# facebookresearch/jepa

Measured on NVIDIA H100. Metric: clips/sec ViT-L/16 16x224^2 synthetic V-JEPA pre-training step, higher is better.
Workload: dtype bf16

## Files before the change

### jepa_b200/csrc/attn_bwd.cu

```cuda
#include <stdlib.h>

#include "attn_common.cuh"
#include "vjepa_b200.h"

namespace vj {

constexpr int kBwdStream = 64;
constexpr int kBwdStages = 3;

struct AttnBwdParams {
  const int* cu_seqlens;
  const float* lse2;
  const float* delta;
  __nv_bfloat16* dqkv;
  int H, T;
  float scale, scale_log2;
};

template <int HD, bool DKV>
constexpr int bwd_nwg() { return HD == 128 || (HD == 64 && DKV) ? 2 : (HD == 32 && !DKV) ? 4 : 3; }

template <int HD, int NWG>
struct BwdCfg {
  using A = AttnCfg<HD>;
  static constexpr int RES = A::template tile_bytes<AttnWarps<NWG>::ROWS>();
  static constexpr int STR = A::template tile_bytes<kBwdStream>();
  static constexpr int T0 = 0, T1 = RES;
  static constexpr int S_OFF = 2 * RES;
  static constexpr int STAT_OFF = S_OFF + kBwdStages * 2 * STR;
  static constexpr int STAT = 2 * kBwdStream * 4;
  static constexpr int BAR_OFF = STAT_OFF + kBwdStages * STAT;
  static constexpr int SMEM_BYTES = BAR_OFF + 8 * (1 + 2 * kBwdStages) + 1024;
  static_assert(SMEM_BYTES <= 232448, "attention backward shared memory budget exceeded");
};

__global__ void __launch_bounds__(256) attn_delta_kernel(const __nv_bfloat16* __restrict__ o,
                                                         const __nv_bfloat16* __restrict__ dout,
                                                         float* __restrict__ delta, int T, int H, int HD) {
  const int lane = threadIdx.x & 31;
  const int wpb = blockDim.x >> 5;
  const int D = H * HD;
  const int nvec = D >> 3;
  const int lanes_per_head = HD >> 3;
  for (long long t = (long long)blockIdx.x * wpb + (threadIdx.x >> 5); t < T; t += (long long)gridDim.x * wpb) {
    for (int c = lane; c < ((nvec + 31) / 32) * 32; c += 32) {
      float s = 0.f;
      if (c < nvec) {
        const uint4 a = *reinterpret_cast<const uint4*>(o + t * D + c * 8);
        const uint4 b = *reinterpret_cast<const uint4*>(dout + t * D + c * 8);
        s = bf16_lo(a.x) * bf16_lo(b.x) + bf16_hi(a.x) * bf16_hi(b.x) + bf16_lo(a.y) * bf16_lo(b.y) +
            bf16_hi(a.y) * bf16_hi(b.y) + bf16_lo(a.z) * bf16_lo(b.z) + bf16_hi(a.z) * bf16_hi(b.z) +
            bf16_lo(a.w) * bf16_lo(b.w) + bf16_hi(a.w) * bf16_hi(b.w);
      }
      for (int o2 = lanes_per_head >> 1; o2 > 0; o2 >>= 1) s += __shfl_xor_sync(0xffffffffu, s, o2);
      if (c < nvec && (lane % lanes_per_head) == 0) delta[(long long)((c * 8) / HD) * T + t] = s;
    }
  }
}

template <int HD, bool DKV, int NWG>
__global__ void __launch_bounds__(AttnWarps<NWG>::THREADS, 1)
attn_bwd_kernel(const __grid_constant__ CUtensorMap tmRes, const __grid_constant__ CUtensorMap tmStr,
                const __grid_constant__ CUtensorMap tmDO, const AttnBwdParams p) {
  using B = BwdCfg<HD, NWG>;
  using W = AttnWarps<NWG>;
  extern __shared__ uint8_t smem_raw[];
  uint8_t* smem = reinterpret_cast<uint8_t*>((reinterpret_cast<uintptr_t>(smem_raw) + 1023) & ~uintptr_t(1023));

  const int seq = blockIdx.y, head = blockIdx.z;
  const int row_begin = p.cu_seqlens[seq];
  const int len = p.cu_seqlens[seq + 1] - row_begin;
  const int t0 = blockIdx.x * W::ROWS;
  if (t0 >= len) return;
  const int n_wg = attn_active_wgs<NWG>(len, t0);
  const int n_it = (len + kBwdStream - 1) / kBwdStream;
  const int HHD = p.H * HD;

  uint64_t* bars = reinterpret_cast<uint64_t*>(smem + B::BAR_OFF);
  const uint32_t bar_res = smem_u32(bars + 0);
  const uint32_t full0 = smem_u32(bars + 1);
  const uint32_t empty0 = smem_u32(bars + 1 + kBwdStages);
  const uint32_t sT0 = smem_u32(smem + B::T0), sT1 = smem_u32(smem + B::T1), sS = smem_u32(smem + B::S_OFF);
  const uint32_t sStat = smem_u32(smem + B::STAT_OFF);
  const float* lse_h = p.lse2 + (long long)head * p.T + row_begin;
  const float* del_h = p.delta + (long long)head * p.T + row_begin;
  const int wg = __shfl_sync(0xffffffffu, threadIdx.x >> 7, 0);
  const int lane = threadIdx.x & 31;

  if (threadIdx.x == 0) {
    mbar_init(bar_res, 1);
    for (int st = 0; st < kBwdStages; ++st) {
      mbar_init(full0 + 8 * st, DKV ? 32 : 1);
      mbar_init(empty0 + 8 * st, 4 * n_wg);
    }
    fence_mbar_init();
  }
  __syncthreads();

  if (wg == 0) {
    setmaxnreg_dec<W::PRODUCER_REGS>();
    if (threadIdx.x < 32) {
      if (lane == 0) {
        mbar_expect_tx(bar_res, 2 * B::RES);
        if (DKV) {
          attn_load_tile<HD, W::ROWS>(sT0, &tmRes, bar_res, HHD + head * HD, row_begin + t0);
          attn_load_tile<HD, W::ROWS>(sT1, &tmRes, bar_res, 2 * HHD + head * HD, row_begin + t0);
        } else {
          attn_load_tile<HD, W::ROWS>(sT0, &tmRes, bar_res, head * HD, row_begin + t0);
          attn_load_tile<HD, W::ROWS>(sT1, &tmDO, bar_res, head * HD, row_begin + t0);
        }
      }
      for (int i = 0; i < n_it; ++i) {
        const int st = i % kBwdStages;
        const uint32_t a = sS + st * 2 * B::STR, b = a + B::STR, bar = full0 + 8 * st;
        const int c0 = i * kBwdStream;
        mbar_wait(empty0 + 8 * st, ((i / kBwdStages) & 1) ^ 1);
        if (DKV) {
#pragma unroll
          for (int k = 0; k < kBwdStream / 32; ++k) {
            const int col = c0 + 32 * k + lane;
            const uint32_t dst = sStat + st * B::STAT + (32 * k + lane) * 4;
            sts32f(dst, col < len ? lse_h[col] : 0.f);
            sts32f(dst + B::STAT / 2, col < len ? del_h[col] : 0.f);
          }
        }
        if (lane == 0) {
          mbar_expect_tx(bar, 2 * B::STR);
          if (DKV) {
            attn_load_tile<HD, kBwdStream>(a, &tmStr, bar, head * HD, row_begin + c0);
            attn_load_tile<HD, kBwdStream>(b, &tmDO, bar, head * HD, row_begin + c0);
          } else {
            attn_load_tile<HD, kBwdStream>(a, &tmStr, bar, HHD + head * HD, row_begin + c0);
            attn_load_tile<HD, kBwdStream>(b, &tmStr, bar, 2 * HHD + head * HD, row_begin + c0);
          }
        } else if (DKV) {
          mbar_arrive(bar);
        }
      }
    }
    return;
  }

  const int cw = wg - 1;
  if (cw >= n_wg) return;
  setmaxnreg_inc<W::CONSUMER_REGS>();
  const int r = cw * 64 + ((threadIdx.x >> 5) & 3) * 16 + (lane >> 2);
  float acc0[HD / 2], acc1[HD / 2];
#pragma unroll
  for (int i = 0; i < HD / 2; ++i) { acc0[i] = 0.f; acc1[i] = 0.f; }
  float row_lse[2], row_del[2];
  if (!DKV) {
#pragma unroll
    for (int h = 0; h < 2; ++h) {
      const int q = t0 + r + 8 * h;
      row_lse[h] = q < len ? lse_h[q] : 0.f;
      row_del[h] = q < len ? del_h[q] : 0.f;
    }
  }
  mbar_wait(bar_res, 0);
  for (int i = 0; i < n_it; ++i) {
    const int st = i % kBwdStages;
    const uint32_t sa = sS + st * 2 * B::STR, sb = sa + B::STR;
    const int c0 = i * kBwdStream;
    mbar_wait(full0 + 8 * st, (i / kBwdStages) & 1);
    float x[kBwdStream / 2], y[kBwdStream / 2];
    wgmma_fence();
#pragma unroll
    for (int kk = 0; kk < HD / 16; ++kk)
      wgmma_ss<kBwdStream, 0, 0>(x, attn_kmajor_desc<HD, W::ROWS>(sT0, cw * 64, kk), attn_kmajor_desc<HD, kBwdStream>(sa, 0, kk),
                                 kk > 0);
#pragma unroll
    for (int kk = 0; kk < HD / 16; ++kk)
      wgmma_ss<kBwdStream, 0, 0>(y, attn_kmajor_desc<HD, W::ROWS>(sT1, cw * 64, kk), attn_kmajor_desc<HD, kBwdStream>(sb, 0, kk),
                                 kk > 0);
    wgmma_commit();
    wgmma_wait<0>();
    wgmma_fence_regs(x);
    wgmma_fence_regs(y);

#pragma unroll
    for (int c = 0; c < kBwdStream / 8; ++c)
#pragma unroll
      for (int e = 0; e < 2; ++e) {
        const int col = 8 * c + 2 * (lane & 3) + e;
        const bool col_ok = c0 + col < len;
        float cl = 0.f, cd = 0.f;
        if (DKV) {
          cl = lds32f(sStat + st * B::STAT + col * 4);
          cd = lds32f(sStat + st * B::STAT + B::STAT / 2 + col * 4);
        }
#pragma unroll
        for (int h = 0; h < 2; ++h) {
          const float l2 = DKV ? cl : row_lse[h], dl = DKV ? cd : row_del[h];
          float& pv = x[4 * c + 2 * h + e];
          float& dv = y[4 * c + 2 * h + e];
          pv = col_ok ? ex2_approx(fmaf(pv, p.scale_log2, -l2)) : 0.f;
          dv = pv * (dv - dl);
        }
      }

    wgmma_fence_regs(acc0);
    wgmma_fence_regs(acc1);
    wgmma_fence();
#pragma unroll
    for (int kk = 0; kk < kBwdStream / 16; ++kk) {
      uint32_t a[4];
      if (DKV) {
        acc_to_afrag(x, kk, a);
        wgmma_rs<HD, 1>(acc0, a, attn_mnmajor_desc<HD, kBwdStream>(sb, kk), 1);
        acc_to_afrag(y, kk, a);
        wgmma_rs<HD, 1>(acc1, a, attn_mnmajor_desc<HD, kBwdStream>(sa, kk), 1);
      } else {
        acc_to_afrag(y, kk, a);
        wgmma_rs<HD, 1>(acc0, a, attn_mnmajor_desc<HD, kBwdStream>(sa, kk), 1);
      }
    }
    wgmma_commit();
    wgmma_wait<0>();
    wgmma_fence_regs(acc0);
    wgmma_fence_regs(acc1);
    __syncwarp();
    if (lane == 0) mbar_arrive(empty0 + 8 * st);
  }

  __nv_bfloat16* rows = p.dqkv + (long long)(row_begin + t0) * 3 * HHD + head * HD;
  if (DKV) {
    store_frag<HD>(acc1, p.scale, rows + HHD, 3LL * HHD, r, len - t0);
    store_frag<HD>(acc0, 1.0f, rows + 2 * HHD, 3LL * HHD, r, len - t0);
  } else {
    store_frag<HD>(acc0, p.scale, rows, 3LL * HHD, r, len - t0);
  }
}

template <int HD>
static int launch_attn_bwd(const void* qkv, const void* out, const void* dout, const float* lse2, float* delta,
                           void* dqkv, const int* cu, int nseq, int max_len, int H, int T, float scale, cudaStream_t s) {
  constexpr int NKV = bwd_nwg<HD, true>(), NQ = bwd_nwg<HD, false>();
  using C = AttnCfg<HD>;
  using BKV = BwdCfg<HD, NKV>;
  using BQ = BwdCfg<HD, NQ>;
  using WKV = AttnWarps<NKV>;
  using WQ = AttnWarps<NQ>;
  CUtensorMap tq_kv, tq_q, tdo_q, tq64, tdo64;
  const uint64_t W = (uint64_t)3 * H * HD, WO = (uint64_t)H * HD;
  int rc = make_tmap_2d(&tq_kv, qkv, 0, W, T, W * 2, C::BOX_INNER, WKV::ROWS, C::TMAP_SWIZZLE);
  if (!rc) rc = make_tmap_2d(&tq_q, qkv, 0, W, T, W * 2, C::BOX_INNER, WQ::ROWS, C::TMAP_SWIZZLE);
  if (!rc) rc = make_tmap_2d(&tq64, qkv, 0, W, T, W * 2, C::BOX_INNER, kBwdStream, C::TMAP_SWIZZLE);
  if (!rc) rc = make_tmap_2d(&tdo_q, dout, 0, WO, T, WO * 2, C::BOX_INNER, WQ::ROWS, C::TMAP_SWIZZLE);
  if (!rc) rc = make_tmap_2d(&tdo64, dout, 0, WO, T, WO * 2, C::BOX_INNER, kBwdStream, C::TMAP_SWIZZLE);
  if (rc) return rc;
  auto kdkv = attn_bwd_kernel<HD, true, NKV>;
  auto kdq = attn_bwd_kernel<HD, false, NQ>;
  static bool configured = false;
  if (!configured) {
    VJ_CUDA(cudaFuncSetAttribute(kdkv, cudaFuncAttributeMaxDynamicSharedMemorySize, BKV::SMEM_BYTES));
    VJ_CUDA(cudaFuncSetAttribute(kdq, cudaFuncAttributeMaxDynamicSharedMemorySize, BQ::SMEM_BYTES));
    configured = true;
  }
  {
    int g = (T + 7) / 8;
    const int cap = num_sms() * 8;
    if (g > cap) g = cap;
    attn_delta_kernel<<<g, 256, 0, s>>>(reinterpret_cast<const __nv_bfloat16*>(out),
                                        reinterpret_cast<const __nv_bfloat16*>(dout), delta, T, H, HD);
    VJ_CUDA(cudaGetLastError());
    vj::count_launch(1);
  }
  AttnBwdParams p;
  p.cu_seqlens = cu; p.lse2 = lse2; p.delta = delta; p.dqkv = reinterpret_cast<__nv_bfloat16*>(dqkv);
  p.H = H; p.T = T; p.scale = scale; p.scale_log2 = scale * 1.4426950408889634f;
  kdkv<<<dim3((max_len + WKV::ROWS - 1) / WKV::ROWS, nseq, H), WKV::THREADS, BKV::SMEM_BYTES, s>>>(tq_kv, tq64, tdo64, p);
  VJ_CUDA(cudaGetLastError());
  kdq<<<dim3((max_len + WQ::ROWS - 1) / WQ::ROWS, nseq, H), WQ::THREADS, BQ::SMEM_BYTES, s>>>(tq_q, tq64, tdo_q, p);
  VJ_CUDA(cudaGetLastError());
  vj::count_launch(2);
  return 0;
}

}

extern "C" int vj_attn_bwd(const void* qkv, const void* out, const void* dout, const float* lse2, float* delta_ws,
                           void* dqkv, float* dq_acc_ws, const int* cu_seqlens, int nseq, int max_len, int H, int HD,
                           int T, float scale, void* stream_) {
  using namespace vj;
  (void)dq_acc_ws;
  cudaStream_t s = reinterpret_cast<cudaStream_t>(stream_);
  VJ_CHECK_ARG(qkv && out && dout && lse2 && delta_ws && dqkv && cu_seqlens, "vj_attn_bwd: null pointer");
  VJ_CHECK_ARG(nseq > 0 && max_len > 0 && H > 0 && T > 0, "vj_attn_bwd: empty problem");
  switch (HD) {
    case 32: return launch_attn_bwd<32>(qkv, out, dout, lse2, delta_ws, dqkv, cu_seqlens, nseq, max_len, H, T, scale, s);
    case 64: return launch_attn_bwd<64>(qkv, out, dout, lse2, delta_ws, dqkv, cu_seqlens, nseq, max_len, H, T, scale, s);
    case 128: return launch_attn_bwd<128>(qkv, out, dout, lse2, delta_ws, dqkv, cu_seqlens, nseq, max_len, H, T, scale, s);
    default: set_error("vj_attn_bwd: head dim %d unsupported (32/64/128)", HD); return -1;
  }
}
```

### jepa_b200/csrc/attn_common.cuh

```cuda
#pragma once
#include "common.cuh"
#include "wgmma.cuh"

namespace vj {

template <int HD>
struct AttnCfg {
  static constexpr int BOX_INNER = HD >= 64 ? 64 : HD;
  static constexpr int NBOX = HD / BOX_INNER;
  static constexpr int ROW_BYTES = BOX_INNER * 2;
  static constexpr int LAYOUT = HD >= 64 ? 1 : 2;
  static constexpr int TMAP_SWIZZLE = HD >= 64 ? 3 : 2;
  static constexpr int SBO = 8 * ROW_BYTES;
  template <int ROWS>
  static constexpr int tile_bytes() { return ROWS * HD * 2; }
};

template <int NWG>
struct AttnWarps {
  static constexpr int THREADS = 128 * (NWG + 1);
  static constexpr int ROWS = 64 * NWG;
  static constexpr int PRODUCER_REGS = NWG == 2 ? 40 : NWG == 3 ? 32 : 24;
  static constexpr int CONSUMER_REGS = NWG == 2 ? 232 : NWG == 3 ? 160 : 112;
  static_assert(NWG >= 2 && NWG <= 4, "2..4 consumer warpgroups");
  static_assert(128 * PRODUCER_REGS + 128 * NWG * CONSUMER_REGS <= (65536 / THREADS) / 8 * 8 * THREADS,
                "setmaxnreg split exceeds the registers allocated at launch");
};

template <int NWG>
VJ_DEVINL int attn_active_wgs(int len, int t0) { return min(NWG, (len - t0 + 63) / 64); }

template <int HD, int ROWS>
VJ_DEVINL uint64_t attn_kmajor_desc(uint32_t tile, int row0, int kk) {
  using C = AttnCfg<HD>;
  constexpr int steps_per_box = C::BOX_INNER / 16;
  const uint32_t addr = tile + (kk / steps_per_box) * (ROWS * C::ROW_BYTES) + row0 * C::ROW_BYTES + (kk % steps_per_box) * 32;
  return make_smem_desc(addr, 16, C::SBO, C::LAYOUT);
}
template <int HD, int ROWS>
VJ_DEVINL uint64_t attn_mnmajor_desc(uint32_t tile, int kk) {
  using C = AttnCfg<HD>;
  return make_smem_desc(tile + kk * 16 * C::ROW_BYTES, ROWS * C::ROW_BYTES, C::SBO, C::LAYOUT);
}

template <int HD, int ROWS>
VJ_DEVINL void attn_load_tile(uint32_t dst, const CUtensorMap* m, uint32_t bar, int c0, int r0) {
  using C = AttnCfg<HD>;
#pragma unroll
  for (int b = 0; b < C::NBOX; ++b) tma_load_2d(dst + b * ROWS * C::ROW_BYTES, m, bar, c0 + b * C::BOX_INNER, r0);
}

template <typename T = __nv_bfloat16, int R>
VJ_DEVINL void acc_to_afrag(const float (&d)[R], int kk, uint32_t (&a)[4]) {
  a[0] = Elt<T>::pack(d[8 * kk + 0], d[8 * kk + 1]);
  a[1] = Elt<T>::pack(d[8 * kk + 2], d[8 * kk + 3]);
  a[2] = Elt<T>::pack(d[8 * kk + 4], d[8 * kk + 5]);
  a[3] = Elt<T>::pack(d[8 * kk + 6], d[8 * kk + 7]);
}

VJ_DEVINL float quad_max(float v) {
  v = fmaxf(v, __shfl_xor_sync(0xffffffffu, v, 1));
  return fmaxf(v, __shfl_xor_sync(0xffffffffu, v, 2));
}
VJ_DEVINL float quad_sum(float v) {
  v += __shfl_xor_sync(0xffffffffu, v, 1);
  return v + __shfl_xor_sync(0xffffffffu, v, 2);
}

template <int HD, typename T = __nv_bfloat16>
VJ_DEVINL void store_frag(const float (&d)[HD / 2], float mul, T* base, long long ld, int r, int rows_valid) {
  const int lane = threadIdx.x & 31;
#pragma unroll
  for (int h = 0; h < 2; ++h) {
    const int row = r + 8 * h;
    if (row >= rows_valid) continue;
#pragma unroll
    for (int j = 0; j < HD / 8; ++j)
      *reinterpret_cast<uint32_t*>(base + (long long)row * ld + 8 * j + 2 * (lane & 3)) =
          Elt<T>::pack(d[4 * j + 2 * h] * mul, d[4 * j + 2 * h + 1] * mul);
  }
}

}
```

Measured before the change: 149.7.

## Overlap attention backward wgmma groups and precompute smem descriptors

Splits the two score GEMMs into separate commit groups so the exp of P can run while the dP GEMM is still in flight. For head dims below 128, the gradient-accumulation wgmma of the current stream tile is left outstanding into the next iteration, and the stage is released one iteration later. It also builds shared-memory descriptors once and advances them by byte offsets, loads the per-column stats as 64-bit pairs, and splits the masked and unmasked exp paths. Keeping the A-fragments live across iterations adds register pressure and delays stage release.

```diff
diff --git a/jepa_b200/csrc/attn_bwd.cu b/jepa_b200/csrc/attn_bwd.cu
--- a/jepa_b200/csrc/attn_bwd.cu
+++ b/jepa_b200/csrc/attn_bwd.cu
@@ -19,6 +19,9 @@
 
 template <int HD, bool DKV>
 constexpr int bwd_nwg() { return HD == 128 || (HD == 64 && DKV) ? 2 : (HD == 32 && !DKV) ? 4 : 3; }
+
+template <int HD, bool DKV>
+constexpr bool kBwdOverlap = HD < 128 && (DKV || HD != 32);
 
 template <int HD, int NWG>
 struct BwdCfg {
@@ -157,70 +160,99 @@
       row_del[h] = q < len ? del_h[q] : 0.f;
     }
   }
+  const uint64_t dT0 = attn_kmajor_desc<HD, W::ROWS>(sT0, cw * 64, 0), dT1 = attn_kmajor_desc<HD, W::ROWS>(sT1, cw * 64, 0);
+  const uint64_t dSk = attn_kmajor_desc<HD, kBwdStream>(sS, 0, 0), dSm = attn_mnmajor_desc<HD, kBwdStream>(sS, 0);
+  uint32_t pf[DKV ? kBwdStream / 16 : 1][4], sf[kBwdStream / 16][4];
+  auto retire = [&](int i) {
+    wgmma_fence_regs(acc0);
+    wgmma_fence_regs(acc1);
+    wgmma_fence_regs(sf);
+    if (DKV) wgmma_fence_regs(pf);
+    __syncwarp();
+    if (lane == 0) mbar_arrive(empty0 + 8 * (i % kBwdStages));
+  };
   mbar_wait(bar_res, 0);
   for (int i = 0; i < n_it; ++i) {
     const int st = i % kBwdStages;
-    const uint32_t sa = sS + st * 2 * B::STR, sb = sa + B::STR;
     const int c0 = i * kBwdStream;
     mbar_wait(full0 + 8 * st, (i / kBwdStages) & 1);
     float x[kBwdStream / 2], y[kBwdStream / 2];
+    const uint32_t oa = st * 2 * B::STR, ob = oa + B::STR;
     wgmma_fence();
 #pragma unroll
     for (int kk = 0; kk < HD / 16; ++kk)
-      wgmma_ss<kBwdStream, 0, 0>(x, attn_kmajor_desc<HD, W::ROWS>(sT0, cw * 64, kk), attn_kmajor_desc<HD, kBwdStream>(sa, 0, kk),
-                                 kk > 0);
+      wgmma_ss<kBwdStream, 0, 0>(x, desc_advance(dT0, attn_kmajor_step<HD, W::ROWS>(kk)),
+                                 desc_advance(dSk, oa + attn_kmajor_step<HD, kBwdStream>(kk)), kk > 0);
+    wgmma_commit();
 #pragma unroll
     for (int kk = 0; kk < HD / 16; ++kk)
-      wgmma_ss<kBwdStream, 0, 0>(y, attn_kmajor_desc<HD, W::ROWS>(sT1, cw * 64, kk), attn_kmajor_desc<HD, kBwdStream>(sb, 0, kk),
-                                 kk > 0);
+      wgmma_ss<kBwdStream, 0, 0>(y, desc_advance(dT1, attn_kmajor_step<HD, W::ROWS>(kk)),
+                                 desc_advance(dSk, ob + attn_kmajor_step<HD, kBwdStream>(kk)), kk > 0);
     wgmma_commit();
+    wgmma_wait<1>();
+    wgmma_fence_regs(x);
+    if (kBwdOverlap<HD, DKV> && i > 0) retire(i - 1);
+
+    const int valid = len - c0;
+    auto exp_p = [&](bool masked) {
+#pragma unroll
+      for (int c = 0; c < kBwdStream / 8; ++c) {
+        const int col = 8 * c + 2 * (lane & 3);
+        const float2 cl = DKV ? lds64f(sStat + st * B::STAT + col * 4) : make_float2(0.f, 0.f);
+#pragma unroll
+        for (int e = 0; e < 2; ++e)
+#pragma unroll
+          for (int h = 0; h < 2; ++h) {
+            float& pv = x[4 * c + 2 * h + e];
+            const float l2 = DKV ? (e ? cl.y : cl.x) : row_lse[h];
+            pv = masked && col + e >= valid ? 0.f : ex2_approx(fmaf(pv, p.scale_log2, -l2));
+          }
+      }
+    };
+    if (valid >= kBwdStream) exp_p(false);
+    else exp_p(true);
+
     wgmma_wait<0>();
-    wgmma_fence_regs(x);
     wgmma_fence_regs(y);
-
-#pragma unroll
-    for (int c = 0; c < kBwdStream / 8; ++c)
-#pragma unroll
-      for (int e = 0; e < 2; ++e) {
-        const int col = 8 * c + 2 * (lane & 3) + e;
-        const bool col_ok = c0 + col < len;
-        float cl = 0.f, cd = 0.f;
-        if (DKV) {
-          cl = lds32f(sStat + st * B::STAT + col * 4);
-          cd = lds32f(sStat + st * B::STAT + B::STAT / 2 + col * 4);
+#pragma unroll
+    for (int c = 0; c < kBwdStream / 8; ++c) {
+      const float2 cd = DKV ? lds64f(sStat + st * B::STAT + B::STAT / 2 + (8 * c + 2 * (lane & 3)) * 4)
+                            : make_float2(0.f, 0.f);
+#pragma unroll
+      for (int e = 0; e < 2; ++e)
+#pragma unroll
+        for (int h = 0; h < 2; ++h) {
+          float& dv = y[4 * c + 2 * h + e];
+          dv = x[4 * c + 2 * h + e] * (dv - (DKV ? (e ? cd.y : cd.x) : row_del[h]));
         }
-#pragma unroll
-        for (int h = 0; h < 2; ++h) {
-          const float l2 = DKV ? cl : row_lse[h], dl = DKV ? cd : row_del[h];
-          float& pv = x[4 * c + 2 * h + e];
-          float& dv = y[4 * c + 2 * h + e];
-          pv = col_ok ? ex2_approx(fmaf(pv, p.scale_log2, -l2)) : 0.f;
-          dv = pv * (dv - dl);
-        }
-      }
-
+    }
+
+#pragma unroll
+    for (int kk = 0; kk < kBwdStream / 16; ++kk) {
+      if (DKV) acc_to_afrag(x, kk, pf[kk]);
+      acc_to_afrag(y, kk, sf[kk]);
+    }
     wgmma_fence_regs(acc0);
     wgmma_fence_regs(acc1);
     wgmma_fence();
 #pragma unroll
     for (int kk = 0; kk < kBwdStream / 16; ++kk) {
-      uint32_t a[4];
       if (DKV) {
-        acc_to_afrag(x, kk, a);
-        wgmma_rs<HD, 1>(acc0, a, attn_mnmajor_desc<HD, kBwdStream>(sb, kk), 1);
-        acc_to_afrag(y, kk, a);
-        wgmma_rs<HD, 1>(acc1, a, attn_mnmajor_desc<HD, kBwdStream>(sa, kk), 1);
+        wgmma_rs<HD, 1>(acc0, pf[kk], desc_advance(dSm, ob + attn_mnmajor_step<HD>(kk)), 1);
+        wgmma_rs<HD, 1>(acc1, sf[kk], desc_advance(dSm, oa + attn_mnmajor_step<HD>(kk)), 1);
       } else {
-        acc_to_afrag(y, kk, a);
-        wgmma_rs<HD, 1>(acc0, a, attn_mnmajor_desc<HD, kBwdStream>(sa, kk), 1);
+        wgmma_rs<HD, 1>(acc0, sf[kk], desc_advance(dSm, oa + attn_mnmajor_step<HD>(kk)), 1);
       }
     }
     wgmma_commit();
+    if (!kBwdOverlap<HD, DKV>) {
+      wgmma_wait<0>();
+      retire(i);
+    }
+  }
+  if (kBwdOverlap<HD, DKV>) {
     wgmma_wait<0>();
-    wgmma_fence_regs(acc0);
-    wgmma_fence_regs(acc1);
-    __syncwarp();
-    if (lane == 0) mbar_arrive(empty0 + 8 * st);
+    retire(n_it - 1);
   }
 
   __nv_bfloat16* rows = p.dqkv + (long long)(row_begin + t0) * 3 * HHD + head * HD;
diff --git a/jepa_b200/csrc/attn_common.cuh b/jepa_b200/csrc/attn_common.cuh
--- a/jepa_b200/csrc/attn_common.cuh
+++ b/jepa_b200/csrc/attn_common.cuh
@@ -31,17 +31,25 @@
 VJ_DEVINL int attn_active_wgs(int len, int t0) { return min(NWG, (len - t0 + 63) / 64); }
 
 template <int HD, int ROWS>
+VJ_DEVINL uint32_t attn_kmajor_step(int kk) {
+  using C = AttnCfg<HD>;
+  constexpr int steps_per_box = C::BOX_INNER / 16;
+  return (kk / steps_per_box) * (ROWS * C::ROW_BYTES) + (kk % steps_per_box) * 32;
+}
+template <int HD>
+VJ_DEVINL uint32_t attn_mnmajor_step(int kk) { return kk * 16 * AttnCfg<HD>::ROW_BYTES; }
+
+template <int HD, int ROWS>
 VJ_DEVINL uint64_t attn_kmajor_desc(uint32_t tile, int row0, int kk) {
   using C = AttnCfg<HD>;
-  constexpr int steps_per_box = C::BOX_INNER / 16;
-  const uint32_t addr = tile + (kk / steps_per_box) * (ROWS * C::ROW_BYTES) + row0 * C::ROW_BYTES + (kk % steps_per_box) * 32;
-  return make_smem_desc(addr, 16, C::SBO, C::LAYOUT);
+  return make_smem_desc(tile + row0 * C::ROW_BYTES + attn_kmajor_step<HD, ROWS>(kk), 16, C::SBO, C::LAYOUT);
 }
 template <int HD, int ROWS>
 VJ_DEVINL uint64_t attn_mnmajor_desc(uint32_t tile, int kk) {
   using C = AttnCfg<HD>;
-  return make_smem_desc(tile + kk * 16 * C::ROW_BYTES, ROWS * C::ROW_BYTES, C::SBO, C::LAYOUT);
+  return make_smem_desc(tile + attn_mnmajor_step<HD>(kk), ROWS * C::ROW_BYTES, C::SBO, C::LAYOUT);
 }
+VJ_DEVINL uint64_t desc_advance(uint64_t desc, uint32_t bytes) { return desc + (bytes >> 4); }
 
 template <int HD, int ROWS>
 VJ_DEVINL void attn_load_tile(uint32_t dst, const CUtensorMap* m, uint32_t bar, int c0, int r0) {
@@ -56,6 +64,12 @@
   a[1] = Elt<T>::pack(d[8 * kk + 2], d[8 * kk + 3]);
   a[2] = Elt<T>::pack(d[8 * kk + 4], d[8 * kk + 5]);
   a[3] = Elt<T>::pack(d[8 * kk + 6], d[8 * kk + 7]);
+}
+
+VJ_DEVINL float2 lds64f(uint32_t addr) {
+  float2 v;
+  asm volatile("ld.shared.v2.f32 {%0, %1}, [%2];" : "=f"(v.x), "=f"(v.y) : "r"(addr) : "memory");
+  return v;
 }
 
 VJ_DEVINL float quad_max(float v) {
```

Result: faster. 151.9, median of 6 (+1.4%).
